# Yan-Xia/Text2Loc

Hardware: AMD Instinct MI355X
Metric: coarse-retrieval queries/sec over 11k-cell DB, embed_dim=256; top-1/3/5 recall parity (higher is better)
Workload: dtype f16; 1 GPU; KITTI360Pose-sized val DB: N=11259 cells x D=256 resident in HBM, Q=4096 precomputed text embeddings per step, top-10 (float64-exact ids); n_cells=11259, embed_dim=256, top_k=10, parallelism=single-gpu, layout=one resident DB, two launches per step (scan, re-rank)

## Files before the change

### text2loc_amd/csrc/capi.hip

```cpp
#include <limits.h>
#include <string.h>

#include "t2l_internal.h"

namespace t2l {

int fail(t2l_ctx* ctx, int code, const std::string& msg) {
  if (ctx) ctx->err = msg;
  return code;
}

void event_begin(t2l_ctx* ctx, const char* name, hipStream_t s) {
  if (!ctx->profile_events) return;
  EventRing& e = ctx->events[name];
  if (e.a.empty()) {
    e.a.resize(kEventRing);
    e.b.resize(kEventRing);
    for (int i = 0; i < kEventRing; ++i) {
      (void)hipEventCreate(&e.a[i]);
      (void)hipEventCreate(&e.b[i]);
    }
  }
  e.open = (e.calls++ % ctx->profile_events) == 0;
  if (e.open) (void)hipEventRecord(e.a[e.head], s);
// ... 315 lines not shown
  }
  return hipSuccess;
}

int t2l_search_fallbacks(t2l_ctx* ctx, int32_t* out_count) {
  if (!ctx || !out_count) return T2L_EINVAL;
  T2L_HIP(ctx, hipSetDevice(ctx->device));
  T2L_HIP(ctx, hipDeviceSynchronize());
  int32_t c[8];
  T2L_HIP(ctx, read_counters(ctx, c));
  *out_count = c[0] + (c[7] - c[6]);
  return T2L_OK;
}

#ifdef T2L_STAMPS
int t2l_debug_stamps(t2l_ctx* ctx, long long* out24) {
  T2L_HIP(ctx, hipDeviceSynchronize());
  T2L_HIP(ctx, hipMemcpy(out24, ctx->fb_count + 16, 24 * sizeof(long long), hipMemcpyDeviceToHost));
  const long long init[8] = {0, 0, 0, 0, LLONG_MAX, 0, LLONG_MAX, 0};
  T2L_HIP(ctx, hipMemcpy(ctx->fb_count + 16, init, sizeof(init), hipMemcpyHostToDevice));
  return T2L_OK;
}
#endif

int t2l_search_counters(t2l_ctx* ctx, int32_t* out8) {
  if (!ctx || !out8) return T2L_EINVAL;
  T2L_HIP(ctx, hipSetDevice(ctx->device));
  T2L_HIP(ctx, hipDeviceSynchronize());
  T2L_HIP(ctx, read_counters(ctx, out8));
  return T2L_OK;
}

int t2l_search_rescored(t2l_ctx* ctx, int32_t* out_count) {
// ... 342 lines not shown
```

### text2loc_amd/csrc/search.hip

```cpp
#include <float.h>
#include <limits.h>

#include <type_traits>

#include "t2l_internal.h"
#include "search_dev.h"

namespace t2l {

__device__ __forceinline__ void reset_counts(int32_t* fb_count, int32_t* fb_prev, int zero_counts, int tid) {
  if (zero_counts && tid < 16) {
    fb_count[64 + tid] = fb_prev[tid];
    fb_prev[tid] = 0;
  }
  if (!zero_counts && tid == 0) {
    fb_count[12] += fb_count[4];
    fb_count[4] = fb_count[6] = 0;
  }
}


__global__ __launch_bounds__(256) void split_db_kernel(const float* __restrict__ db, uint4* __restrict__ out, int rows) {
  const int gid = blockIdx.x * 256 + threadIdx.x;
  const int row = gid >> 5, c = gid & 31;
  if (row >= rows) return;
  const float4* src = reinterpret_cast<const float4*>(db + (size_t)row * kD + 8 * c);
  uint4 hi, lo;
  split8(src[0], src[1], hi, lo);
  out[(size_t)row * 64 + c] = hi;
  out[(size_t)row * 64 + 32 + c] = lo;
}

constexpr int kWideQPerWave = 64;
constexpr int kWideQPerBlock = 4 * kWideQPerWave;

template <int LL, int NBUF>
__global__ __launch_bounds__(256, 1) void scanw_kernel(const uint4* __restrict__ dbs, int n_rows, int n_tiles, int code_bits,
                                                       const float* __restrict__ q, int Q, int nsplit,
                                                       float* __restrict__ cand, int32_t* __restrict__ fb_count, int32_t* __restrict__ fb_prev,
                                                       int zero_counts, float pinf) {
  extern __shared__ __attribute__((aligned(16))) float smem[];
  const int tid = threadIdx.x, lane = tid & 63, wave = tid >> 6;
  const int half = lane >> 5, col = lane & 31;
  const int sp = blockIdx.x % nsplit, qb = blockIdx.x / nsplit;
  const int nt = sp < n_tiles ? (n_tiles - sp + nsplit - 1) / nsplit : 0;
  const int qrow0 = qb * kWideQPerBlock + wave * kWideQPerWave + col, qrow1 = qrow0 + 32;
  const int mask = ~((1 << code_bits) - 1);
  int vmask = mask;
  asm volatile("" : "+v"(vmask));
  if (blockIdx.x == 0) reset_counts(fb_count, fb_prev, zero_counts, tid);
  if (nt == 0) return;
  const int uwave = uniform_wave_id();

  auto dma_of = [&](int j, int buf) {
    const int tile = sp + min(j, nt - 1) * nsplit;
    WideDma d;
    d.src = reinterpret_cast<const char*>(dbs) + ((size_t)tile * kTileRows + uwave * 8) * 1024;
    d.dst = lds_addr_of(smem + buf * kTileFloats + uwave * 8 * kRowStrideF);
    d.lane16 = lane * 16;
    return d;
  };
#pragma unroll
  for (int b = 0; b < NBUF - 1; ++b) {
    const WideDma d = dma_of(b, b);
#pragma unroll
// ... 84 lines not shown
  if (pos >= rows_pad) return;
  const int row = plane_row(pos, n_rows);
  if (row >= n_rows) {
    out[gid] = make_uint4(0u, 0u, 0u, 0u);
    return;
  }
  int shift;
  half_shift_of(norms[1], shift);
  const float4* src = reinterpret_cast<const float4*>(db + (size_t)row * kD + 8 * c);
  const float4 a = src[0], b = src[1];
  out[gid] = make_uint4(pack_f16x2(a.x, a.y, shift), pack_f16x2(a.z, a.w, shift), pack_f16x2(b.x, b.y, shift),
                        pack_f16x2(b.z, b.w, shift));
}

template <int LL>
__global__ __launch_bounds__(256, 1) void scanh_kernel(const uint4* __restrict__ dbh, int n_rows, int n_tiles, int code_bits,
                                                       const float* __restrict__ q, int Q, int nsplit,
                                                       float* __restrict__ cand, int32_t* __restrict__ fb_count, int32_t* __restrict__ fb_prev,
                                                       int zero_counts, float pinf) {
  constexpr int NBUF = 4;
  extern __shared__ __attribute__((aligned(16))) float smem[];
  const int tid = threadIdx.x, lane = tid & 63;
  const int half = lane >> 5, col = lane & 31;
  const int sp = blockIdx.x % nsplit, qb = blockIdx.x / nsplit;
  const int nt = sp < n_tiles ? (n_tiles - sp + nsplit - 1) / nsplit : 0;
  const int uwave = uniform_wave_id();
  const int qrow0 = qb * kWideQPerBlock + uwave * kWideQPerWave + col, qrow1 = qrow0 + 32;
  const int mask = ~((1 << code_bits) - 1);
  int vmask = mask;
  asm volatile("" : "+v"(vmask));
  if (blockIdx.x == 0) reset_counts(fb_count, fb_prev, zero_counts, tid);
  if (nt == 0) return;

  const unsigned lds_base = lds_addr_of(smem);
  auto dma_of = [&](int j, int buf) {
    const int tile = sp + min(j, nt - 1) * nsplit;
    HalfDma d;
    d.src = reinterpret_cast<const char*>(dbh) + (size_t)tile * kHalfTileBytes + uwave * 4096;
    d.dst = lds_base + buf * kHalfTileBytes + uwave * 4096;
    d.lane16 = lane * 16;
    return d;
  };
#pragma unroll
  for (int b = 0; b < NBUF - 1; ++b) {
    const HalfDma d = dma_of(b, b);
#pragma unroll
// ... 100 lines not shown
  double* out_score;
  int32_t* flags;
  int32_t* fb_count;
  float eps_rel_probe, pinf;
  int n_rows, defer, stat_mode;
  int32_t* host_stat;
  int seq, wide_cap;
  int rec6;
  int slot_bits = 0;
};

constexpr int kMergedLL = 8;
#ifndef T2L_SEL_RD
#define T2L_SEL_RD 2
#endif
template <int LL, int NS, bool MERGE = false, int SEL = 0>
__global__ __launch_bounds__(512, 1) void scanp_kernel(const uint4* __restrict__ dbt, int n_rows, int n_tiles, int code_bits,
                                                       const float* __restrict__ q, int Q, int nsplit,
                                                       float* __restrict__ cand, int32_t* __restrict__ fb_count, int32_t* __restrict__ fb_prev,
                                                       int zero_counts, float pinf, unsigned long long* __restrict__ span,
                                                       unsigned span_seq, int xcd_qgroups, int slot_bits) {
  static_assert(NS == 4, "the step loop below is unrolled for a ring of 4 slots");
  constexpr bool EPI = SEL == 1;
  static_assert(!MERGE || LL == 6, "the in-workgroup list merge is written for lists of 6");
  static_assert(!SEL || MERGE, "the tile-local selection's dropped-bound leaves through the merged record's bound");
  extern __shared__ __attribute__((aligned(16))) float smem[];
  constexpr int kSlotBytes = 2 * kHalfTileBytes;
  constexpr unsigned kExchange = 2 * kSlotBytes;
  const int tid = threadIdx.x, lane = tid & 63;
  const int half = lane >> 5, col = lane & 31;
  int sp = blockIdx.x % nsplit, qb = blockIdx.x / nsplit;
  if (xcd_qgroups > 1) {
    const int GQ = xcd_qgroups, GS = 8 / GQ, nqb = gridDim.x / nsplit;
    const int x = blockIdx.x & 7, j = blockIdx.x >> 3, per = nqb / GQ;
    qb = (j % per) * GQ + x % GQ;
    sp = (j / per) * GS + x / GQ;
  }
  const int uwave = uniform_wave_id();
  const int quad = uwave >> 2, wq = uwave & 3;
  const int vn = 2 * nsplit, vs = sp + quad * nsplit;
  const int nt = vs < n_tiles ? (n_tiles - vs + vn - 1) / vn : 0;
  const int steps = sp < n_tiles ? (n_tiles - sp + vn - 1) / vn : 0;
  constexpr int kCS = MERGE ? 2 : 0;
  const int mask = ~((1 << (code_bits + kCS)) - 1);
  const int code_q = MERGE ? (quad << 1) : 0;
  int vmask = mask;
  asm volatile("" : "+v"(vmask));
  if (blockIdx.x == 0) reset_counts(fb_count, fb_prev, zero_counts, tid);
  if (steps == 0) return;
  const unsigned long long wg_t0 = __builtin_amdgcn_s_memrealtime();
#ifdef T2L_STAMPS
#define T2L_STAMP(k)                                                                                                   \
  if (tid == 0) {                                                                                                      \
    const long long t_ = __builtin_amdgcn_s_memrealtime();                                                             \
    if (blockIdx.x == 37) reinterpret_cast<long long*>(fb_count + 16)[k] = t_;                                         \
    if (k == 0) atomicMin(reinterpret_cast<unsigned long long*>(fb_count + 16) + 4, (unsigned long long)t_);           \
    if (k == 0) atomicMax(reinterpret_cast<unsigned long long*>(fb_count + 16) + 5, (unsigned long long)t_);           \
    if (k == 3) atomicMin(reinterpret_cast<unsigned long long*>(fb_count + 16) + 6, (unsigned long long)t_);           \
    if (k == 3) atomicMax(reinterpret_cast<unsigned long long*>(fb_count + 16) + 7, (unsigned long long)t_);           \
  }
#define T2L_STAMP2(k) if (tid == 0 && blockIdx.x == 37) reinterpret_cast<long long*>(fb_count + 32)[k] = __builtin_amdgcn_s_memrealtime()
#define T2L_STAMP3(k)                                                                                                  \
  {                                                                                                                    \
    __builtin_amdgcn_sched_barrier(0);                                                                                 \
    if (tid == 0 && blockIdx.x == 37) reinterpret_cast<long long*>(fb_count + 48)[k] = __builtin_amdgcn_s_memrealtime(); \
    __builtin_amdgcn_sched_barrier(0);                                                                                 \
  }
#else
#define T2L_STAMP(k)
#define T2L_STAMP2(k)
#define T2L_STAMP3(k)
#endif
  T2L_STAMP(0);

  const unsigned lds_base = lds_addr_of(smem);
  const unsigned lane16 = lane * 16;
  auto dma_of = [&](int i, int slot) {
    PairDma d;
    const int t0 = min(sp + (2 * i) * nsplit, n_tiles - 1), t1 = min(sp + (2 * i + 1) * nsplit, n_tiles - 1);
    d.src0 = reinterpret_cast<const char*>(dbt) + (size_t)t0 * kHalfTileBytes + uwave * 2048;
    d.src1 = reinterpret_cast<const char*>(dbt) + (size_t)t1 * kHalfTileBytes + uwave * 2048;
    d.dst = lds_base + slot * kSlotBytes + uwave * 2048;
    d.lane16 = lane16;
    return d;
  };
#pragma unroll
  for (int b = 0; b < 2; ++b) {
    const PairDma d = dma_of(b, b);
#pragma unroll
    for (int e = 0; e < 4; ++e) d.piece(e);
  }

  u32x4 q0[16], q1[16];
  {
    const int ql = tid >> 2, qt = tid & 3;
    char* ex_w = reinterpret_cast<char*>(smem) + kExchange + ql * 512;
    const char* ex_r = reinterpret_cast<const char*>(smem) + kExchange + (wq * 32 + col) * 512;
    float4 v[2][16];
#pragma unroll
    for (int g = 0; g < 2; ++g) {
      const int qrow = min(qb * kWideQPerBlock + (ql >> 5) * kWideQPerWave + g * 32 + (ql & 31), Q - 1);
      const float4* qp = reinterpret_cast<const float4*>(q + (size_t)qrow * kD) + qt;
#pragma unroll
      for (int i = 0; i < 16; ++i) v[g][i] = qp[4 * i];
#ifdef T2L_EXP_HALFLOAD
      if (g == 1) {
#pragma unroll
        for (int i = 0; i < 16; ++i) v[1][i] = v[0][i];
      }
#endif
    }
#pragma unroll
    for (int g = 0; g < 2; ++g) {
      float m = 0.f;
#pragma unroll
      for (int i = 0; i < 16; ++i) {
        m = fmaxf(fmaxf(m, fabsf(v[g][i].x)), fabsf(v[g][i].y));
        m = fmaxf(fmaxf(m, fabsf(v[g][i].z)), fabsf(v[g][i].w));
      }
      if (g == 0) { T2L_STAMP2(0); } else { T2L_STAMP2(3); }
      m = fmaxf(m, dpp_f<kDppXor1>(m));
      m = fmaxf(m, dpp_f<kDppXor2>(m));
      int shift;
      half_shift_of(m, shift);
      if (g == 1) __syncthreads();
#pragma unroll
      for (int j = 0; j < 16; ++j) {
        const float4 a = v[g][j];
        typedef unsigned u32x2 __attribute__((ext_vector_type(2)));
        *reinterpret_cast<u32x2*>(ex_w + (((2 * j + (qt >> 1)) ^ (ql & 31)) << 4) + ((qt & 1) << 3)) =
            u32x2{pack_f16x2(a.x, a.y, shift), pack_f16x2(a.z, a.w, shift)};
      }
      __syncthreads();
      if (g == 0) { T2L_STAMP2(1); } else { T2L_STAMP2(4); }
#pragma unroll
      for (int s = 0; s < 16; ++s) {
        const u32x4 f = *reinterpret_cast<const u32x4*>(ex_r + ((((half << 4) + s) ^ col) << 4));
        if (g == 0) q0[s] = pin_agpr(f); else q1[s] = pin_agpr(f);
      }
      if (g == 0) { T2L_STAMP2(2); } else { T2L_STAMP2(5); }
    }
    __syncthreads();
  }
  T2L_STAMP(1);
  {
    const PairDma d = dma_of(2, 2);
#pragma unroll
    for (int e = 0; e < 4; ++e) d.piece(e);
  }

  std::conditional_t<SEL != 0, TileSelLists<LL>, WideLists<LL>> w;
#pragma unroll
  for (int i = 0; i < LL; ++i) w.ls0[i] = w.ls1[i] = T2L_NEG_INF;
  if constexpr (SEL) w.dA0 = w.dB0 = w.dA1 = w.dB1 = w.t0 = w.t1 = w.t2 = w.k = T2L_NEG_INF;
  else w.key0 = w.key1 = T2L_NEG_INF;
  f32x16 accA0, accA1, accB0, accB1;
#pragma unroll
  for (int r = 0; r < 16; ++r) accA0[r] = accA1[r] = accB0[r] = accB1[r] = T2L_NEG_INF;
// ... 192 lines not shown
      T2L_STAMP3(5);
      const int qrow = qb * kWideQPerBlock + wq * kWideQPerWave + lane;
      if (qrow < Q) {
        float4* out = reinterpret_cast<float4*>(cand + ((size_t)qrow * nsplit + record_slot(sp, nsplit, slot_bits)) * kMergedLL);
        out[0] = make_float4(M[0], M[1], M[2], M[3]);
        out[1] = make_float4(M[4], M[5], M[6], M[7]);
      }
      T2L_STAMP3(6);
    }
  } else {
    put_list(qrow0, w.ls0);
    put_list(qrow1, w.ls1);
  }
  if (span && threadIdx.x == 0) {
    const unsigned long long t1 = __builtin_amdgcn_s_memrealtime(), tag = (unsigned long long)span_seq << 40, tm = (1ull << 40) - 1;
    *reinterpret_cast<ulonglong2*>(span + 2 * blockIdx.x) = make_ulonglong2(tag | (wg_t0 & tm), tag | (t1 & tm));
  }
  T2L_STAMP(3);
}

template <int NW>
struct WgExactSharedN {
  double score[NW][32];
  int row[NW][32];
};
typedef WgExactSharedN<4> WgExactShared;

constexpr int kWideCap = 1024;

__device__ __forceinline__ void top32_insert(double& ts, int& tr, double cd, int cr, int lane) {
  {
// ... 109 lines not shown

__device__ __forceinline__ void publish_report(const RerankArgs& a) {
  int32_t* fb_count = a.fb_count;
  if (a.host_stat && a.seq > 0) {
    a.host_stat[1] = fb_count[64 + 10] == 2 ? fb_count[64 + 3] : fb_count[64 + 2];
    a.host_stat[2] = fb_count[64 + 9];
    a.host_stat[3] = fb_count[64 + 0] + fb_count[64 + 4] + fb_count[64 + 12];
    a.host_stat[4] = fb_count[64 + 10];
    a.host_stat[5] = fb_count[64 + 10] == 2 ? fb_count[64 + 3] : fb_count[64 + 1];
    __hip_atomic_store(&a.host_stat[0], a.seq, __ATOMIC_RELEASE, __HIP_MEMORY_SCOPE_SYSTEM);
  }
  fb_count[9] = a.Q;
  fb_count[10] = a.stat_mode;
}

template <int LL, int L, bool MG = false>
__device__ __forceinline__ void rerank_query(const RerankArgs& a, const int qid, const int lane, int* my_wg_flag, int* wr_buf) {
  static_assert(!MG || LL == kMergedLL, "merged records are 8 floats");
  const float* __restrict__ db = a.db;
  const float* __restrict__ q = a.q;
  const int Q = a.Q, K = a.K, parts = a.parts, code_bits = a.code_bits, row_offset = a.row_offset, half_mode = a.half_mode;
  const int slack_bits = MG ? code_bits + 2 : code_bits;
  const int strided_rows = half_mode ? a.n_rows : 0;
  auto krow = [&](float key, int part) {
    if constexpr (MG) {
      const int b = __float_as_int(key), src = b & 3;
      return key_row(__int_as_float(b >> 2), 2 * (part + (src >> 1) * parts) + (src & 1), 2 * parts, code_bits, strided_rows);
    } else {
      return key_row(key, part, parts >> 1, code_bits, strided_rows);
    }
  };
  const float* __restrict__ cand = a.cand;
  const float eps_rel = a.eps_rel, eps_rel_probe = a.eps_rel_probe, pinf = a.pinf;
  const float* __restrict__ db_norm_max = a.db_norm_max;
  int32_t* __restrict__ out_idx = a.out_idx;
  double* __restrict__ out_score = a.out_score;
  int32_t* __restrict__ flags = a.flags;
  int32_t* __restrict__ fb_count = a.fb_count;
  const int n_rows = a.n_rows, defer = a.defer, wide_cap = a.wide_cap;

  float lst[LL];
  {
    const int mslot = MG ? record_slot(min(lane, parts - 1), parts, a.slot_bits) : min(lane, parts - 1);
    const float* mine = cand + ((size_t)qid * parts + mslot) * LL;
    if constexpr (MG) {
      const float4 v0 = reinterpret_cast<const float4*>(mine)[0], v1 = reinterpret_cast<const float4*>(mine)[1];
      lst[0] = v0.x; lst[1] = v0.y; lst[2] = v0.z; lst[3] = v0.w;
      lst[4] = v1.x; lst[5] = v1.y; lst[6] = v1.z; lst[7] = v1.w;
    } else if constexpr (LL % 2 == 0) {
#pragma unroll
      for (int i = 0; i < LL / 2; ++i) {
        const float2 v = reinterpret_cast<const float2*>(mine)[i];
        lst[2 * i] = v.x;
        lst[2 * i + 1] = v.y;
      }
    } else {
#pragma unroll
      for (int i = 0; i < LL; ++i) lst[i] = mine[i];
    }
    if (lane >= parts) {
#pragma unroll
      for (int i = 0; i < LL; ++i) lst[i] = T2L_NEG_INF;
    }
  }
  const float lane_floor = lst[LL - 1];
  if constexpr (MG) lst[LL - 1] = T2L_NEG_INF;
  float b1 = T2L_NEG_INF;
  if constexpr (MG) {
    if (a.rec6) {
      b1 = lst[LL - 2];
      lst[LL - 2] = T2L_NEG_INF;
    }
  }
  const float floor_max = wave_max_f32(fmaxf(lane_floor, b1), pinf);
  const int seg = lane & 15;
  double qd[16];
  float q_absmax = 0.f;
  {
    const float4* qp = reinterpret_cast<const float4*>(q + (size_t)qid * kD) + seg;
#pragma unroll
    for (int i = 0; i < 4; ++i) {
      const float4 v = qp[16 * i];
      qd[4 * i] = (double)v.x;
      qd[4 * i + 1] = (double)v.y;
      qd[4 * i + 2] = (double)v.z;
      qd[4 * i + 3] = (double)v.w;
      q_absmax = fmaxf(fmaxf(fmaxf(q_absmax, fabsf(v.x)), fabsf(v.y)), fmaxf(fabsf(v.z), fabsf(v.w)));
    }
  }

  float my_key = T2L_NEG_INF;
  int my_part = 0;
  auto merge_round = [&](int r) {
    const float bk = wave_max_f32(lst[0], pinf);
    const unsigned long long who = __ballot(lst[0] == bk);
    const int bl = __ffsll((long long)who) - 1;
    if (lane == r) {
      my_key = bk;
      my_part = bl;
    }
    const bool pop = lane == bl;
#pragma unroll
    for (int i = 0; i < LL - 1; ++i) lst[i] = pop ? lst[i + 1] : lst[i];
    lst[LL - 1] = pop ? T2L_NEG_INF : lst[LL - 1];
  };
#pragma unroll
  for (int r = 0; r < L - 4; ++r) merge_round(r);
  int my_row = (lane < L - 4 && my_key != T2L_NEG_INF) ? krow(my_key, my_part) : INT_MAX;

  double kscale = 1.0;
  bool representable = true;
  {
    const float m = row16_max_f32(q_absmax);
    int sq, sd;
    representable = half_shift_of(m, sq);
    representable = half_shift_of(db_norm_max[1], sd) && representable;
    if (half_mode) {
      kscale = ldexp(1.0, -(sq + sd));
    } else {
      representable = representable && abs(sq - 14) <= 40 && abs(sd - 14) <= 40;
    }
  }

  double qn = 0.0;
#pragma unroll
  for (int i = 0; i < 16; ++i) qn += qd[i] * qd[i];
  qn = row16_sum_f64(qn);
  const double eps32 = (double)eps_rel * sqrt(qn) * (double)(*db_norm_max);
  constexpr int LA = L - 4;
  float4 rows[L / 4][4];
  auto gather = [&](int p) {
    const int row = __shfl(my_row, 4 * p + (lane >> 4));
#ifdef T2L_EXP_RERANK_TWICE
    {
      const int other = row == INT_MAX ? 0 : (row * 7 + 13) % n_rows;
      const float4* op = reinterpret_cast<const float4*>(db + (size_t)other * kD) + seg;
#pragma unroll
      for (int i = 0; i < 4; ++i) {
        float4 v = op[16 * i];
        asm volatile("" ::"v"(v.x), "v"(v.y), "v"(v.z), "v"(v.w));
      }
    }
#endif
    const float4* rp = reinterpret_cast<const float4*>(db + (size_t)(row == INT_MAX ? 0 : row) * kD) + seg;
#pragma unroll
    for (int i = 0; i < 4; ++i) rows[p][i] = rp[16 * i];
  };
  double my_d = -__builtin_inf();
  auto score = [&](int p) {
    double d0 = 0.0, d1 = 0.0;
#pragma unroll
    for (int i = 0; i < 4; ++i) {
      d0 += (double)rows[p][i].x * qd[4 * i];
      d1 += (double)rows[p][i].y * qd[4 * i + 1];
      d0 += (double)rows[p][i].z * qd[4 * i + 2];
      d1 += (double)rows[p][i].w * qd[4 * i + 3];
    }
    const double d = row16_sum_f64(d0 + d1);
    const double mine = __shfl(d, 16 * (lane & 3));
    if ((lane >> 2) == p && lane < L && my_row != INT_MAX) my_d = mine;
  };
  auto rank_among = [&](auto n_tag) {
// ... 7 lines not shown
      const int ij = __builtin_amdgcn_readlane(my_row, j);
      r += (dj > my_d || (dj == my_d && ij < my_row)) ? 1 : 0;
    }
    return r;
  };
  auto emit = [&](bool ok, int r) {
    if (lane < K) {
      out_idx[(size_t)qid * K + lane] = -1;
      if (out_score) out_score[(size_t)qid * K + lane] = -__builtin_inf();
    }
    if (ok && r < K) {
      out_idx[(size_t)qid * K + r] = my_row + row_offset;
      if (out_score) out_score[(size_t)qid * K + r] = my_d;
    }
  };
#pragma unroll
  for (int p = 0; p < L / 4 - 1; ++p) gather(p);
#pragma unroll
  for (int p = 0; p < L / 4 - 1; ++p) score(p);
  bool early = false;
  if (K <= LA && representable && eps_rel_probe == 0.f) {
    const float gA = fmaxf(__uint_as_float(__builtin_amdgcn_readlane(__float_as_uint(my_key), LA - 1)), floor_max);
    if (gA != T2L_NEG_INF) {
      const int rA = rank_among(std::integral_constant<int, LA>{});
      const bool validA = lane < LA && my_row != INT_MAX;
      const unsigned long long kthA = __ballot(validA && rA == K - 1);
      if (kthA != 0ull) {
        const double dK = __shfl(my_d, __ffsll((long long)kthA) - 1);
        if (dK > (double)gA * kscale + key_slack(gA, slack_bits, eps32, kscale)) {
          emit(validA, rA);
          early = true;
        }
// ... 295 lines not shown
    }
  }
  }
  }
}

template <int LL, int L, bool MG = false>
__global__ __launch_bounds__(256, (MG ? 4 : 1)) void rerank_kernel(const float* __restrict__ db, const float* __restrict__ q, int Q,
                                                     int K, int parts, int code_bits,
                                                     const float* __restrict__ cand, int row_offset, float eps_rel,
                                                     const float* __restrict__ db_norm_max, int half_mode,
                                                     int32_t* __restrict__ out_idx, double* __restrict__ out_score,
                                                     int32_t* __restrict__ flags, int32_t* __restrict__ fb_count,
                                                     float eps_rel_probe, float pinf, int n_rows, int defer, int stat_mode,
                                                     int32_t* __restrict__ host_stat, int seq, int wide_cap, int rec6, int slot_bits) {
  __shared__ WgExactShared exact_sh;
  __shared__ int wg_flag[4];
  __shared__ int wide_rows[4][kWideCap];
  const RerankArgs a{db, q, Q, K, parts, code_bits, cand, row_offset, eps_rel, db_norm_max, half_mode, out_idx, out_score, flags, fb_count,
                     eps_rel_probe, pinf, n_rows, defer, stat_mode, host_stat, seq, wide_cap, rec6, slot_bits};
  const int lane = threadIdx.x & 63;
  const int qid = blockIdx.x * 4 + (threadIdx.x >> 6);
  if (threadIdx.x < 4) wg_flag[threadIdx.x] = 0;
  if (blockIdx.x == 0 && threadIdx.x == 0) publish_report(a);
  __syncthreads();
  if (qid < Q) rerank_query<LL, L, MG>(a, qid, lane, &wg_flag[threadIdx.x >> 6], wide_rows[threadIdx.x >> 6]);
  __syncthreads();
#pragma unroll 1
  for (int w = 0; w < 4; ++w) {
    if (!wg_flag[w]) continue;
    const int fq = blockIdx.x * 4 + w;
    if (threadIdx.x == 0) atomicAdd(&fb_count[0], 1);
    wg_exact_scan(db, n_rows, q + (size_t)fq * kD, K, row_offset, out_idx + (size_t)fq * K,
                  out_score ? out_score + (size_t)fq * K : nullptr, exact_sh);
  }
}

__global__ __launch_bounds__(256) void db_norm_kernel(const float* __restrict__ db, int n_rows, float* out) {
  __shared__ float red[4];
  __shared__ int red_a[4];
  const int lane = threadIdx.x & 63, wave = threadIdx.x >> 6;
// ... 93 lines not shown
                         bool first, bool pair, hipStream_t s) {
  const int n_tiles = (n_rows + kTileRows - 1) / kTileRows;
  const int parts = 2 * nsplit;
  const int zero = first;
  const int half_mode = ctx->eff_mode == 0;
  const bool probing = ctx->search_mode == 0 && ctx->eff_mode == 2;
  const double operand_eps = ctx->eff_mode == 0 ? 9.85e-4 : (ctx->eff_mode == 2 ? 2.0e-5 : 0.0);
  const float eps_rel = (float)(ctx->eps_scale * ((kD + 8) * 5.9604644775390625e-08 + operand_eps));
  const float eps_probe = probing ? (float)(ctx->eps_scale * ((kD + 8) * 5.9604644775390625e-08 + 9.85e-4)) : 0.f;
  const int stat_mode = probing ? 2 : (half_mode ? 1 : 0);
  const int seq = first ? ++ctx->stat_seq : 0;
  const int defer = ctx->heavy ? 1 : 0;
  bool merged = false;
  int rec_slot_bits = 0;
  if constexpr (LL <= 6) {
    const dim3 grid((Q + kWideQPerBlock - 1) / kWideQPerBlock * (nsplit / 2));
    const size_t lds = (size_t)4 * 2 * kHalfTileBytes + (size_t)256 * (kMergedLL + 3) * sizeof(float);
    static PerDeviceOnce once;
    if (once.need(ctx->device)) {
      allow_lds(&scanp_kernel<LL, 4>, lds);
      if constexpr (LL == 6) allow_lds(&scanp_kernel<LL, 4, true>, lds);
      if constexpr (LL == 6) allow_lds(&scanp_kernel<LL, 4, true, 1>, lds);
      if constexpr (LL == 6) allow_lds(&scanp_kernel<LL, 4, true, 2>, lds);
      once.mark(ctx->device);
    }
    const unsigned span_seq = ++ctx->span_seq;
    unsigned long long* span = ctx->scan_span && grid.x <= (unsigned)kSpanWgs ? ctx->scan_span + (size_t)2 * kSpanWgs * (span_seq % kSpanRing) : nullptr;
    if (ctx->span_grid) ctx->span_grid[span_seq % kSpanRing] = span ? grid.x : 0;
    int xq = ctx->xcd_qgroups;
    {
      const int nqb = (Q + kWideQPerBlock - 1) / kWideQPerBlock, ns = nsplit / 2;
      if (xq < 2 || 8 % xq || nqb % xq || ns % (8 / xq) || (nqb * ns) % 8) xq = 1;
    }
    int slot_bits = 0;
    if (ctx->search_epilogue && xq > 1)
      for (int gs = 8 / xq; gs > 1; gs >>= 1) ++slot_bits;
    rec_slot_bits = slot_bits;
    hipEvent_t ea, eb;
    const bool ev = event_pair(ctx, "search_scan", &ea, &eb);
    auto launch = [&](auto kern) {
      if (ev)
        hipExtLaunchKernelGGL(kern, grid, dim3(512), (uint32_t)lds, s, ea, eb, 0u, dbh, n_rows, n_tiles, code_bits, q, Q, nsplit / 2, ctx->cand_score,
                              ctx->fb_count, ctx->fb_prev, zero, __builtin_inff(), span, span_seq, xq, slot_bits);
      else
        hipLaunchKernelGGL(kern, grid, dim3(512), lds, s, dbh, n_rows, n_tiles, code_bits, q, Q, nsplit / 2, ctx->cand_score, ctx->fb_count,
                           ctx->fb_prev, zero, __builtin_inff(), span, span_seq, xq, slot_bits);
    };
    if constexpr (LL == 6 && L == 16) {
      merged = (ctx->search_merge == 1 || (ctx->search_merge == 2 && ctx->merge_live && !ctx->heavy)) && code_bits <= 9;
    }
    if constexpr (LL == 6) {
      if (merged && ctx->search_tile_sel && ctx->search_epilogue) launch(scanp_kernel<LL, 4, true, 1>);
      else if (merged && ctx->search_tile_sel) launch(scanp_kernel<LL, 4, true, 2>);
      else if (merged) launch(scanp_kernel<LL, 4, true>);
    }
    if (!merged) launch(scanp_kernel<LL, 4>);
  } else {
  event_begin(ctx, "search_scan", s);
  if (ctx->eff_mode == 0) {
    const dim3 grid((Q + kWideQPerBlock - 1) / kWideQPerBlock * nsplit);
    const size_t lds = (size_t)4 * kHalfTileBytes;
    static PerDeviceOnce once;
    if (once.need(ctx->device)) {
      allow_lds(&scanh_kernel<LL>, (size_t)4 * kHalfTileBytes);
      once.mark(ctx->device);
    }
    hipLaunchKernelGGL((scanh_kernel<LL>), grid, dim3(256), lds, s, dbh, n_rows, n_tiles, code_bits, q, Q, nsplit,
                       ctx->cand_score, ctx->fb_count, ctx->fb_prev, zero, __builtin_inff());
  } else if (ctx->eff_mode == 2) {
    const dim3 grid((Q + kWideQPerBlock - 1) / kWideQPerBlock * nsplit);
    const size_t lds = (size_t)4 * kTileFloats * sizeof(float);
    static PerDeviceOnce once;
    if (once.need(ctx->device)) {
      allow_lds(&scanw_kernel<LL, 4>, (size_t)4 * kTileFloats * sizeof(float));
      once.mark(ctx->device);
    }
    hipLaunchKernelGGL((scanw_kernel<LL, 4>), grid, dim3(256), lds, s, dbs, n_rows, n_tiles, code_bits, q, Q, nsplit,
                       ctx->cand_score, ctx->fb_count, ctx->fb_prev, zero, __builtin_inff());
  }
  event_end(ctx, "search_scan", s);
  }
  T2L_HIP(ctx, hipGetLastError());
  hipEvent_t ea, eb;
  if constexpr (LL == 6 && L == 16) {
    if (merged) {
      const bool evr = ctx->profile_rerank && event_pair(ctx, "search_rerank", &ea, &eb);
      if (evr)
        hipExtLaunchKernelGGL((rerank_kernel<kMergedLL, L, true>), dim3((Q + 3) / 4), dim3(256), 0u, s, ea, eb, 0u, db, q, Q, K, nsplit / 2,
                              code_bits, (const float*)ctx->cand_score, row_offset, eps_rel, (const float*)ctx->db_norm_max, half_mode, out_idx,
                              out_score, ctx->flags, ctx->fb_count, eps_probe, __builtin_inff(), n_rows, defer, stat_mode,
                              ctx->host_stat_dev, seq, min(ctx->wide_repair, kWideCap), ctx->search_tile_sel ? 1 : 0, rec_slot_bits);
      else
// ... 226 lines not shown
```

### text2loc_amd/csrc/search_dev.h

```cpp
#pragma once
#include <float.h>
#include <limits.h>

#include "t2l_internal.h"

namespace t2l {

typedef float f32x16 __attribute__((ext_vector_type(16)));

#define T2L_NEG_INF (-__builtin_inff())

template <int L, int I = L - 1>
__device__ __forceinline__ void ins_key(float (&s)[L], float x) {
  if constexpr (I == 0) {
    s[0] = __builtin_amdgcn_fmed3f(s[0], x, __builtin_inff());
  } else {
    s[I] = __builtin_amdgcn_fmed3f(s[I - 1], s[I], x);
    ins_key<L, I - 1>(s, x);
  }
}

__device__ __forceinline__ float make_key(float v, int mask, int code) {
  return __int_as_float((__float_as_int(v) & mask) | code);
}
// ... 489 lines not shown
```

Baseline: 101.1 million queries/s.

## Overlap scan prologue loads, use 2D/3D grids, and prefetch rerank inputs early

The scan kernels now take a 2D or 3D grid with precomputed tiles-per-split quotient and remainder, which removes the per-block integer division and modulo and the XCD remapping arithmetic. The merged scan kernel issues query loads with explicit vmcnt waits, half of them into AGPRs, interleaved with the first DB tile DMAs, and it defers the counter reset until after that prologue. The rerank kernel prefetches the query row and norm values alongside the candidate lists, drops the leading __syncthreads, and moves publish_report after the per-query work. Optional timestamp instrumentation is also added. The hand-written waitcnt values and AGPR placement are fragile if the instruction mix changes.

```diff
diff --git a/text2loc_amd/csrc/capi.hip b/text2loc_amd/csrc/capi.hip
--- a/text2loc_amd/csrc/capi.hip
+++ b/text2loc_amd/csrc/capi.hip
@@ -353,9 +353,9 @@
 }
 
 #ifdef T2L_STAMPS
-int t2l_debug_stamps(t2l_ctx* ctx, long long* out24) {
+int t2l_debug_stamps(t2l_ctx* ctx, long long* out48) {
   T2L_HIP(ctx, hipDeviceSynchronize());
-  T2L_HIP(ctx, hipMemcpy(out24, ctx->fb_count + 16, 24 * sizeof(long long), hipMemcpyDeviceToHost));
+  T2L_HIP(ctx, hipMemcpy(out48, ctx->fb_count + 16, 48 * sizeof(long long), hipMemcpyDeviceToHost));
   const long long init[8] = {0, 0, 0, 0, LLONG_MAX, 0, LLONG_MAX, 0};
   T2L_HIP(ctx, hipMemcpy(ctx->fb_count + 16, init, sizeof(init), hipMemcpyHostToDevice));
   return T2L_OK;
diff --git a/text2loc_amd/csrc/search.hip b/text2loc_amd/csrc/search.hip
--- a/text2loc_amd/csrc/search.hip
+++ b/text2loc_amd/csrc/search.hip
@@ -35,20 +35,20 @@
 constexpr int kWideQPerBlock = 4 * kWideQPerWave;
 
 template <int LL, int NBUF>
-__global__ __launch_bounds__(256, 1) void scanw_kernel(const uint4* __restrict__ dbs, int n_rows, int n_tiles, int code_bits,
+__global__ __launch_bounds__(256, 1) void scanw_kernel(const uint4* __restrict__ dbs, int n_rows, int tiles_q, int tiles_r, int code_bits,
                                                        const float* __restrict__ q, int Q, int nsplit,
                                                        float* __restrict__ cand, int32_t* __restrict__ fb_count, int32_t* __restrict__ fb_prev,
                                                        int zero_counts, float pinf) {
   extern __shared__ __attribute__((aligned(16))) float smem[];
   const int tid = threadIdx.x, lane = tid & 63, wave = tid >> 6;
   const int half = lane >> 5, col = lane & 31;
-  const int sp = blockIdx.x % nsplit, qb = blockIdx.x / nsplit;
-  const int nt = sp < n_tiles ? (n_tiles - sp + nsplit - 1) / nsplit : 0;
+  const int sp = blockIdx.x, qb = blockIdx.y;
+  const int nt = tiles_q + (sp < tiles_r ? 1 : 0);
   const int qrow0 = qb * kWideQPerBlock + wave * kWideQPerWave + col, qrow1 = qrow0 + 32;
   const int mask = ~((1 << code_bits) - 1);
   int vmask = mask;
   asm volatile("" : "+v"(vmask));
-  if (blockIdx.x == 0) reset_counts(fb_count, fb_prev, zero_counts, tid);
+  if ((blockIdx.x | blockIdx.y) == 0) reset_counts(fb_count, fb_prev, zero_counts, tid);
   if (nt == 0) return;
   const int uwave = uniform_wave_id();
 
@@ -163,7 +163,7 @@
 }
 
 template <int LL>
-__global__ __launch_bounds__(256, 1) void scanh_kernel(const uint4* __restrict__ dbh, int n_rows, int n_tiles, int code_bits,
+__global__ __launch_bounds__(256, 1) void scanh_kernel(const uint4* __restrict__ dbh, int n_rows, int tiles_q, int tiles_r, int code_bits,
                                                        const float* __restrict__ q, int Q, int nsplit,
                                                        float* __restrict__ cand, int32_t* __restrict__ fb_count, int32_t* __restrict__ fb_prev,
                                                        int zero_counts, float pinf) {
@@ -171,14 +171,14 @@
   extern __shared__ __attribute__((aligned(16))) float smem[];
   const int tid = threadIdx.x, lane = tid & 63;
   const int half = lane >> 5, col = lane & 31;
-  const int sp = blockIdx.x % nsplit, qb = blockIdx.x / nsplit;
-  const int nt = sp < n_tiles ? (n_tiles - sp + nsplit - 1) / nsplit : 0;
+  const int sp = blockIdx.x, qb = blockIdx.y;
+  const int nt = tiles_q + (sp < tiles_r ? 1 : 0);
   const int uwave = uniform_wave_id();
   const int qrow0 = qb * kWideQPerBlock + uwave * kWideQPerWave + col, qrow1 = qrow0 + 32;
   const int mask = ~((1 << code_bits) - 1);
   int vmask = mask;
   asm volatile("" : "+v"(vmask));
-  if (blockIdx.x == 0) reset_counts(fb_count, fb_prev, zero_counts, tid);
+  if ((blockIdx.x | blockIdx.y) == 0) reset_counts(fb_count, fb_prev, zero_counts, tid);
   if (nt == 0) return;
 
   const unsigned lds_base = lds_addr_of(smem);
@@ -309,12 +309,39 @@
 #ifndef T2L_SEL_RD
 #define T2L_SEL_RD 2
 #endif
+#ifdef T2L_STAMPS
+#define T2L_STAMP(k)                                                                                                   \
+  if (tid == 0) {                                                                                                      \
+    const long long t_ = __builtin_amdgcn_s_memrealtime();                                                             \
+    if (wg == 37) reinterpret_cast<long long*>(fb_count + 16)[k] = t_;                                                 \
+    if (k == 0) atomicMin(reinterpret_cast<unsigned long long*>(fb_count + 16) + 4, (unsigned long long)t_);           \
+    if (k == 0) atomicMax(reinterpret_cast<unsigned long long*>(fb_count + 16) + 5, (unsigned long long)t_);           \
+    if (k == 3) atomicMin(reinterpret_cast<unsigned long long*>(fb_count + 16) + 6, (unsigned long long)t_);           \
+    if (k == 3) atomicMax(reinterpret_cast<unsigned long long*>(fb_count + 16) + 7, (unsigned long long)t_);           \
+  }
+#define T2L_STAMP2(k) if (tid == 0 && wg == 37) reinterpret_cast<long long*>(fb_count + 32)[k] = __builtin_amdgcn_s_memrealtime()
+#define T2L_STAMP2_AT(k, t) if (tid == 0 && wg == 37) reinterpret_cast<long long*>(fb_count + 32)[k] = (long long)(t)
+#define T2L_STAMP3(k)                                                                                                  \
+  {                                                                                                                    \
+    __builtin_amdgcn_sched_barrier(0);                                                                                 \
+    if (tid == 0 && wg == 37) reinterpret_cast<long long*>(fb_count + 48)[k] = __builtin_amdgcn_s_memrealtime();       \
+    __builtin_amdgcn_sched_barrier(0);                                                                                 \
+  }
+#else
+#define T2L_STAMP(k)
+#define T2L_STAMP2(k)
+#define T2L_STAMP2_AT(k, t)
+#define T2L_STAMP3(k)
+#endif
+
 template <int LL, int NS, bool MERGE = false, int SEL = 0>
-__global__ __launch_bounds__(512, 1) void scanp_kernel(const uint4* __restrict__ dbt, int n_rows, int n_tiles, int code_bits,
-                                                       const float* __restrict__ q, int Q, int nsplit,
-                                                       float* __restrict__ cand, int32_t* __restrict__ fb_count, int32_t* __restrict__ fb_prev,
-                                                       int zero_counts, float pinf, unsigned long long* __restrict__ span,
-                                                       unsigned span_seq, int xcd_qgroups, int slot_bits) {
+__global__ __launch_bounds__(512, 1) void scanp_kernel(const float* __restrict__ q, const uint4* __restrict__ dbt, int Q, int nsplit,
+                                                       int tiles_q, int tiles_r, int n_tiles, int lgq, int grid_y, int code_bits,
+                                                       int zero_counts, float pinf, int n_rows, unsigned span_seq, int slot_bits,
+                                                       float* __restrict__ cand, int32_t* __restrict__ fb_count,
+                                                       int32_t* __restrict__ fb_prev, unsigned long long* __restrict__ span) {
+  const unsigned long long wg_t0 = __builtin_amdgcn_s_memrealtime();
+  asm volatile("" ::"s"(dbt), "s"(q), "s"(grid_y));
   static_assert(NS == 4, "the step loop below is unrolled for a ring of 4 slots");
   constexpr bool EPI = SEL == 1;
   static_assert(!MERGE || LL == 6, "the in-workgroup list merge is written for lists of 6");
@@ -324,49 +351,20 @@
   constexpr unsigned kExchange = 2 * kSlotBytes;
   const int tid = threadIdx.x, lane = tid & 63;
   const int half = lane >> 5, col = lane & 31;
-  int sp = blockIdx.x % nsplit, qb = blockIdx.x / nsplit;
-  if (xcd_qgroups > 1) {
-    const int GQ = xcd_qgroups, GS = 8 / GQ, nqb = gridDim.x / nsplit;
-    const int x = blockIdx.x & 7, j = blockIdx.x >> 3, per = nqb / GQ;
-    qb = (j % per) * GQ + x % GQ;
-    sp = (j / per) * GS + x / GQ;
-  }
+  const int qb = (blockIdx.y << lgq) + (blockIdx.x & ((1 << lgq) - 1));
+  const int sp = blockIdx.z * (8 >> lgq) + (blockIdx.x >> lgq);
+  const int wg = blockIdx.x + (lgq ? 8 : nsplit) * (blockIdx.y + grid_y * blockIdx.z);
   const int uwave = uniform_wave_id();
   const int quad = uwave >> 2, wq = uwave & 3;
   const int vn = 2 * nsplit, vs = sp + quad * nsplit;
-  const int nt = vs < n_tiles ? (n_tiles - vs + vn - 1) / vn : 0;
-  const int steps = sp < n_tiles ? (n_tiles - sp + vn - 1) / vn : 0;
+  const int nt = tiles_q + (vs < tiles_r ? 1 : 0);
+  const int steps = tiles_q + (sp < tiles_r ? 1 : 0);
   constexpr int kCS = MERGE ? 2 : 0;
   const int mask = ~((1 << (code_bits + kCS)) - 1);
   const int code_q = MERGE ? (quad << 1) : 0;
   int vmask = mask;
   asm volatile("" : "+v"(vmask));
-  if (blockIdx.x == 0) reset_counts(fb_count, fb_prev, zero_counts, tid);
   if (steps == 0) return;
-  const unsigned long long wg_t0 = __builtin_amdgcn_s_memrealtime();
-#ifdef T2L_STAMPS
-#define T2L_STAMP(k)                                                                                                   \
-  if (tid == 0) {                                                                                                      \
-    const long long t_ = __builtin_amdgcn_s_memrealtime();                                                             \
-    if (blockIdx.x == 37) reinterpret_cast<long long*>(fb_count + 16)[k] = t_;                                         \
-    if (k == 0) atomicMin(reinterpret_cast<unsigned long long*>(fb_count + 16) + 4, (unsigned long long)t_);           \
-    if (k == 0) atomicMax(reinterpret_cast<unsigned long long*>(fb_count + 16) + 5, (unsigned long long)t_);           \
-    if (k == 3) atomicMin(reinterpret_cast<unsigned long long*>(fb_count + 16) + 6, (unsigned long long)t_);           \
-    if (k == 3) atomicMax(reinterpret_cast<unsigned long long*>(fb_count + 16) + 7, (unsigned long long)t_);           \
-  }
-#define T2L_STAMP2(k) if (tid == 0 && blockIdx.x == 37) reinterpret_cast<long long*>(fb_count + 32)[k] = __builtin_amdgcn_s_memrealtime()
-#define T2L_STAMP3(k)                                                                                                  \
-  {                                                                                                                    \
-    __builtin_amdgcn_sched_barrier(0);                                                                                 \
-    if (tid == 0 && blockIdx.x == 37) reinterpret_cast<long long*>(fb_count + 48)[k] = __builtin_amdgcn_s_memrealtime(); \
-    __builtin_amdgcn_sched_barrier(0);                                                                                 \
-  }
-#else
-#define T2L_STAMP(k)
-#define T2L_STAMP2(k)
-#define T2L_STAMP3(k)
-#endif
-  T2L_STAMP(0);
 
   const unsigned lds_base = lds_addr_of(smem);
   const unsigned lane16 = lane * 16;
@@ -379,34 +377,48 @@
     d.lane16 = lane16;
     return d;
   };
-#pragma unroll
-  for (int b = 0; b < 2; ++b) {
-    const PairDma d = dma_of(b, b);
-#pragma unroll
-    for (int e = 0; e < 4; ++e) d.piece(e);
-  }
-
   u32x4 q0[16], q1[16];
+  int parked;
   {
     const int ql = tid >> 2, qt = tid & 3;
     char* ex_w = reinterpret_cast<char*>(smem) + kExchange + ql * 512;
     const char* ex_r = reinterpret_cast<const char*>(smem) + kExchange + (wq * 32 + col) * 512;
-    float4 v[2][16];
+    f32x4 v[2][16];
+    auto load_q = [&](auto agpr_tag, f32x4& dst, const float4* p, auto off_tag) {
+      constexpr int OFF = decltype(off_tag)::value;
+      if constexpr (decltype(agpr_tag)::value) asm volatile("global_load_dwordx4 %0, %1, off offset:%2" : "=a"(dst) : "v"(p), "n"(OFF) : "memory");
+      else asm volatile("global_load_dwordx4 %0, %1, off offset:%2" : "=&v"(dst) : "v"(p), "n"(OFF) : "memory");
+    };
+    auto row_ptr = [&](int g) {
+      const int qrow = min(qb * kWideQPerBlock + (ql >> 5) * kWideQPerWave + g * 32 + (ql & 31), Q - 1);
+      return reinterpret_cast<const float4*>(q + (size_t)qrow * kD) + qt;
+    };
+    const float4 *qp0 = row_ptr(0), *qp1 = row_ptr(1);
+    T2L_STAMP(0);
+    static_for<0, 16>([&](auto i) { load_q(std::false_type{}, v[0][i], qp0, std::integral_constant<int, 64 * decltype(i)::value>{}); });
+#pragma unroll
+    for (int b = 0; b < 2; ++b) {
+      const PairDma d = dma_of(b, b);
+#pragma unroll
+      for (int e = 0; e < 4; ++e) d.piece(e);
+    }
+    static_for<0, 16>([&](auto i) { load_q(std::true_type{}, v[1][i], qp1, std::integral_constant<int, 64 * decltype(i)::value>{}); });
+    parked = fb_prev[tid & 15];
+    auto landed = [&](int g) {
+      if (g == 0) {
+        asm volatile("s_waitcnt vmcnt(25)" ::: "memory");
+#pragma unroll
+        for (int i = 0; i < 16; ++i) asm volatile("" : "+v"(v[0][i]));
+      } else {
+        asm volatile("s_waitcnt vmcnt(0)" ::: "memory");
+#pragma unroll
+        for (int i = 0; i < 16; ++i) asm volatile("" : "+a"(v[1][i]));
+        asm volatile("" : "+v"(parked));
+      }
+    };
 #pragma unroll
     for (int g = 0; g < 2; ++g) {
-      const int qrow = min(qb * kWideQPerBlock + (ql >> 5) * kWideQPerWave + g * 32 + (ql & 31), Q - 1);
-      const float4* qp = reinterpret_cast<const float4*>(q + (size_t)qrow * kD) + qt;
-#pragma unroll
-      for (int i = 0; i < 16; ++i) v[g][i] = qp[4 * i];
-#ifdef T2L_EXP_HALFLOAD
-      if (g == 1) {
-#pragma unroll
-        for (int i = 0; i < 16; ++i) v[1][i] = v[0][i];
-      }
-#endif
-    }
-#pragma unroll
-    for (int g = 0; g < 2; ++g) {
+      landed(g);
       float m = 0.f;
 #pragma unroll
       for (int i = 0; i < 16; ++i) {
@@ -421,7 +433,7 @@
       if (g == 1) __syncthreads();
 #pragma unroll
       for (int j = 0; j < 16; ++j) {
-        const float4 a = v[g][j];
+        const f32x4 a = v[g][j];
         typedef unsigned u32x2 __attribute__((ext_vector_type(2)));
         *reinterpret_cast<u32x2*>(ex_w + (((2 * j + (qt >> 1)) ^ (ql & 31)) << 4) + ((qt & 1) << 3)) =
             u32x2{pack_f16x2(a.x, a.y, shift), pack_f16x2(a.z, a.w, shift)};
@@ -437,6 +449,14 @@
     }
     __syncthreads();
   }
+  if (wg == 0) {
+    if (zero_counts && tid < 16) {
+      fb_count[64 + tid] = parked;
+      fb_prev[tid] = 0;
+    }
+    if (!zero_counts) reset_counts(fb_count, fb_prev, 0, tid);
+  }
+  T2L_STAMP2_AT(6, wg_t0);
   T2L_STAMP(1);
   {
     const PairDma d = dma_of(2, 2);
@@ -659,7 +679,7 @@
   }
   if (span && threadIdx.x == 0) {
     const unsigned long long t1 = __builtin_amdgcn_s_memrealtime(), tag = (unsigned long long)span_seq << 40, tm = (1ull << 40) - 1;
-    *reinterpret_cast<ulonglong2*>(span + 2 * blockIdx.x) = make_ulonglong2(tag | (wg_t0 & tm), tag | (t1 & tm));
+    *reinterpret_cast<ulonglong2*>(span + 2 * wg) = make_ulonglong2(tag | (wg_t0 & tm), tag | (t1 & tm));
   }
   T2L_STAMP(3);
 }
@@ -799,6 +819,21 @@
   fb_count[10] = a.stat_mode;
 }
 
+#ifdef T2L_STAMPS
+constexpr int kRerankStampWg = 513;
+#define T2L_RSTAMP_AT(k, t) if (qid == 4 * kRerankStampWg && lane == 0) reinterpret_cast<long long*>(a.fb_count + 96)[k] = (long long)(t)
+#define T2L_RSTAMP(k, ...)                                                                                              \
+  {                                                                                                                    \
+    __builtin_amdgcn_sched_barrier(0);                                                                                 \
+    asm volatile(__VA_ARGS__);                                                                                         \
+    T2L_RSTAMP_AT(k, __builtin_amdgcn_s_memrealtime());                                                                \
+    __builtin_amdgcn_sched_barrier(0);                                                                                 \
+  }
+#else
+#define T2L_RSTAMP_AT(k, t)
+#define T2L_RSTAMP(k, ...)
+#endif
+
 template <int LL, int L, bool MG = false>
 __device__ __forceinline__ void rerank_query(const RerankArgs& a, const int qid, const int lane, int* my_wg_flag, int* wr_buf) {
   static_assert(!MG || LL == kMergedLL, "merged records are 8 floats");
@@ -825,9 +860,13 @@
   const int n_rows = a.n_rows, defer = a.defer, wide_cap = a.wide_cap;
 
   float lst[LL];
+  const int seg = lane & 15;
+  float4 qraw[4];
+  float db_norm, db_absmax;
   {
     const int mslot = MG ? record_slot(min(lane, parts - 1), parts, a.slot_bits) : min(lane, parts - 1);
     const float* mine = cand + ((size_t)qid * parts + mslot) * LL;
+    const float4* qp = reinterpret_cast<const float4*>(q + (size_t)qid * kD) + seg;
     if constexpr (MG) {
       const float4 v0 = reinterpret_cast<const float4*>(mine)[0], v1 = reinterpret_cast<const float4*>(mine)[1];
       lst[0] = v0.x; lst[1] = v0.y; lst[2] = v0.z; lst[3] = v0.w;
@@ -843,6 +882,13 @@
 #pragma unroll
       for (int i = 0; i < LL; ++i) lst[i] = mine[i];
     }
+#pragma unroll
+    for (int i = 0; i < 4; ++i) qraw[i] = qp[16 * i];
+    db_norm = db_norm_max[0];
+    db_absmax = db_norm_max[1];
+    __builtin_amdgcn_sched_barrier(0);
+    T2L_RSTAMP(1, "");
+    T2L_RSTAMP(2, "s_waitcnt vmcnt(%0)" ::"n"(4));
     if (lane >= parts) {
 #pragma unroll
       for (int i = 0; i < LL; ++i) lst[i] = T2L_NEG_INF;
@@ -858,22 +904,6 @@
     }
   }
   const float floor_max = wave_max_f32(fmaxf(lane_floor, b1), pinf);
-  const int seg = lane & 15;
-  double qd[16];
-  float q_absmax = 0.f;
-  {
-    const float4* qp = reinterpret_cast<const float4*>(q + (size_t)qid * kD) + seg;
-#pragma unroll
-    for (int i = 0; i < 4; ++i) {
-      const float4 v = qp[16 * i];
-      qd[4 * i] = (double)v.x;
-      qd[4 * i + 1] = (double)v.y;
-      qd[4 * i + 2] = (double)v.z;
-      qd[4 * i + 3] = (double)v.w;
-      q_absmax = fmaxf(fmaxf(fmaxf(q_absmax, fabsf(v.x)), fabsf(v.y)), fmaxf(fabsf(v.z), fabsf(v.w)));
-    }
-  }
-
   float my_key = T2L_NEG_INF;
   int my_part = 0;
   auto merge_round = [&](int r) {
@@ -893,44 +923,65 @@
   for (int r = 0; r < L - 4; ++r) merge_round(r);
   int my_row = (lane < L - 4 && my_key != T2L_NEG_INF) ? krow(my_key, my_part) : INT_MAX;
 
+  T2L_RSTAMP(3, "");
+  constexpr int LA = L - 4;
+  float4 rows[L / 4][4];
+  auto gather = [&](int p) {
+    const int r0 = __builtin_amdgcn_readlane(my_row, 4 * p), r1 = __builtin_amdgcn_readlane(my_row, 4 * p + 1);
+    const int r2 = __builtin_amdgcn_readlane(my_row, 4 * p + 2), r3 = __builtin_amdgcn_readlane(my_row, 4 * p + 3);
+    const int grp = lane >> 4;
+    const int row = grp == 0 ? r0 : (grp == 1 ? r1 : (grp == 2 ? r2 : r3));
+#ifdef T2L_EXP_RERANK_TWICE
+    {
+      const int other = row == INT_MAX ? 0 : (row * 7 + 13) % n_rows;
+      const float4* op = reinterpret_cast<const float4*>(db + (size_t)other * kD) + seg;
+#pragma unroll
+      for (int i = 0; i < 4; ++i) {
+        float4 v = op[16 * i];
+        asm volatile("" ::"v"(v.x), "v"(v.y), "v"(v.z), "v"(v.w));
+      }
+    }
+#endif
+    const float4* rp = reinterpret_cast<const float4*>(db + (size_t)(row == INT_MAX ? 0 : row) * kD) + seg;
+#pragma unroll
+    for (int i = 0; i < 4; ++i) rows[p][i] = rp[16 * i];
+  };
+#pragma unroll
+  for (int p = 0; p < L / 4 - 1; ++p) {
+    gather(p);
+    if (p == 0) { T2L_RSTAMP(4, ""); }
+  }
+  __builtin_amdgcn_sched_barrier(0);
+
+  double qd[16];
+  float q_absmax = 0.f;
+#pragma unroll
+  for (int i = 0; i < 4; ++i) {
+    const float4 v = qraw[i];
+    qd[4 * i] = (double)v.x;
+    qd[4 * i + 1] = (double)v.y;
+    qd[4 * i + 2] = (double)v.z;
+    qd[4 * i + 3] = (double)v.w;
+    q_absmax = fmaxf(fmaxf(fmaxf(q_absmax, fabsf(v.x)), fabsf(v.y)), fmaxf(fabsf(v.z), fabsf(v.w)));
+  }
   double kscale = 1.0;
   bool representable = true;
   {
     const float m = row16_max_f32(q_absmax);
     int sq, sd;
     representable = half_shift_of(m, sq);
-    representable = half_shift_of(db_norm_max[1], sd) && representable;
+    representable = half_shift_of(db_absmax, sd) && representable;
     if (half_mode) {
       kscale = ldexp(1.0, -(sq + sd));
     } else {
       representable = representable && abs(sq - 14) <= 40 && abs(sd - 14) <= 40;
     }
   }
-
   double qn = 0.0;
 #pragma unroll
   for (int i = 0; i < 16; ++i) qn += qd[i] * qd[i];
   qn = row16_sum_f64(qn);
-  const double eps32 = (double)eps_rel * sqrt(qn) * (double)(*db_norm_max);
-  constexpr int LA = L - 4;
-  float4 rows[L / 4][4];
-  auto gather = [&](int p) {
-    const int row = __shfl(my_row, 4 * p + (lane >> 4));
-#ifdef T2L_EXP_RERANK_TWICE
-    {
-      const int other = row == INT_MAX ? 0 : (row * 7 + 13) % n_rows;
-      const float4* op = reinterpret_cast<const float4*>(db + (size_t)other * kD) + seg;
-#pragma unroll
-      for (int i = 0; i < 4; ++i) {
-        float4 v = op[16 * i];
-        asm volatile("" ::"v"(v.x), "v"(v.y), "v"(v.z), "v"(v.w));
-      }
-    }
-#endif
-    const float4* rp = reinterpret_cast<const float4*>(db + (size_t)(row == INT_MAX ? 0 : row) * kD) + seg;
-#pragma unroll
-    for (int i = 0; i < 4; ++i) rows[p][i] = rp[16 * i];
-  };
+  const double eps32 = (double)eps_rel * sqrt(qn) * (double)db_norm;
   double my_d = -__builtin_inf();
   auto score = [&](int p) {
     double d0 = 0.0, d1 = 0.0;
@@ -968,8 +1019,7 @@
       if (out_score) out_score[(size_t)qid * K + r] = my_d;
     }
   };
-#pragma unroll
-  for (int p = 0; p < L / 4 - 1; ++p) gather(p);
+  T2L_RSTAMP(5, "s_waitcnt vmcnt(%0)" ::"n"(4 * (L / 4 - 2)));
 #pragma unroll
   for (int p = 0; p < L / 4 - 1; ++p) score(p);
   bool early = false;
@@ -1295,6 +1345,9 @@
                                                      int32_t* __restrict__ flags, int32_t* __restrict__ fb_count,
                                                      float eps_rel_probe, float pinf, int n_rows, int defer, int stat_mode,
                                                      int32_t* __restrict__ host_stat, int seq, int wide_cap, int rec6, int slot_bits) {
+#ifdef T2L_STAMPS
+  const long long t_entry = __builtin_amdgcn_s_memrealtime();
+#endif
   __shared__ WgExactShared exact_sh;
   __shared__ int wg_flag[4];
   __shared__ int wide_rows[4][kWideCap];
@@ -1302,10 +1355,12 @@
                      eps_rel_probe, pinf, n_rows, defer, stat_mode, host_stat, seq, wide_cap, rec6, slot_bits};
   const int lane = threadIdx.x & 63;
   const int qid = blockIdx.x * 4 + (threadIdx.x >> 6);
-  if (threadIdx.x < 4) wg_flag[threadIdx.x] = 0;
+  asm volatile("" ::"s"(q), "s"(cand), "s"(db_norm_max), "s"(half_mode));
+  if (lane == 0) wg_flag[threadIdx.x >> 6] = 0;
+  T2L_RSTAMP_AT(0, t_entry);
+  if (qid < Q) rerank_query<LL, L, MG>(a, qid, lane, &wg_flag[threadIdx.x >> 6], wide_rows[threadIdx.x >> 6]);
+  T2L_RSTAMP(6, "");
   if (blockIdx.x == 0 && threadIdx.x == 0) publish_report(a);
-  __syncthreads();
-  if (qid < Q) rerank_query<LL, L, MG>(a, qid, lane, &wg_flag[threadIdx.x >> 6], wide_rows[threadIdx.x >> 6]);
   __syncthreads();
 #pragma unroll 1
   for (int w = 0; w < 4; ++w) {
@@ -1429,7 +1484,8 @@
   bool merged = false;
   int rec_slot_bits = 0;
   if constexpr (LL <= 6) {
-    const dim3 grid((Q + kWideQPerBlock - 1) / kWideQPerBlock * (nsplit / 2));
+    const int nqb = (Q + kWideQPerBlock - 1) / kWideQPerBlock, ns = nsplit / 2;
+    const unsigned n_wgs = (unsigned)(nqb * ns);
     const size_t lds = (size_t)4 * 2 * kHalfTileBytes + (size_t)256 * (kMergedLL + 3) * sizeof(float);
     static PerDeviceOnce once;
     if (once.need(ctx->device)) {
@@ -1440,13 +1496,15 @@
       once.mark(ctx->device);
     }
     const unsigned span_seq = ++ctx->span_seq;
-    unsigned long long* span = ctx->scan_span && grid.x <= (unsigned)kSpanWgs ? ctx->scan_span + (size_t)2 * kSpanWgs * (span_seq % kSpanRing) : nullptr;
-    if (ctx->span_grid) ctx->span_grid[span_seq % kSpanRing] = span ? grid.x : 0;
+    unsigned long long* span = ctx->scan_span && n_wgs <= (unsigned)kSpanWgs ? ctx->scan_span + (size_t)2 * kSpanWgs * (span_seq % kSpanRing) : nullptr;
+    if (ctx->span_grid) ctx->span_grid[span_seq % kSpanRing] = span ? n_wgs : 0;
     int xq = ctx->xcd_qgroups;
-    {
-      const int nqb = (Q + kWideQPerBlock - 1) / kWideQPerBlock, ns = nsplit / 2;
-      if (xq < 2 || 8 % xq || nqb % xq || ns % (8 / xq) || (nqb * ns) % 8) xq = 1;
-    }
+    if (xq < 2 || 8 % xq || nqb % xq || ns % (8 / xq) || (nqb * ns) % 8) xq = 1;
+    int lgq = 0;
+    while ((1 << lgq) < xq) ++lgq;
+    const dim3 grid = xq > 1 ? dim3(8, nqb / xq, ns / (8 / xq)) : dim3(ns, nqb, 1);
+    if (grid.y > 65535u || grid.z > 65535u) return fail(ctx, T2L_EINVAL, "t2l_search: more than 65,535 query blocks in one call");
+    const int vn = 2 * ns, tiles_q = n_tiles / vn, tiles_r = n_tiles % vn;
     int slot_bits = 0;
     if (ctx->search_epilogue && xq > 1)
       for (int gs = 8 / xq; gs > 1; gs >>= 1) ++slot_bits;
@@ -1455,11 +1513,11 @@
     const bool ev = event_pair(ctx, "search_scan", &ea, &eb);
     auto launch = [&](auto kern) {
       if (ev)
-        hipExtLaunchKernelGGL(kern, grid, dim3(512), (uint32_t)lds, s, ea, eb, 0u, dbh, n_rows, n_tiles, code_bits, q, Q, nsplit / 2, ctx->cand_score,
-                              ctx->fb_count, ctx->fb_prev, zero, __builtin_inff(), span, span_seq, xq, slot_bits);
+        hipExtLaunchKernelGGL(kern, grid, dim3(512), (uint32_t)lds, s, ea, eb, 0u, q, dbh, Q, ns, tiles_q, tiles_r, n_tiles, lgq, (int)grid.y,
+                              code_bits, zero, __builtin_inff(), n_rows, span_seq, slot_bits, ctx->cand_score, ctx->fb_count, ctx->fb_prev, span);
       else
-        hipLaunchKernelGGL(kern, grid, dim3(512), lds, s, dbh, n_rows, n_tiles, code_bits, q, Q, nsplit / 2, ctx->cand_score, ctx->fb_count,
-                           ctx->fb_prev, zero, __builtin_inff(), span, span_seq, xq, slot_bits);
+        hipLaunchKernelGGL(kern, grid, dim3(512), lds, s, q, dbh, Q, ns, tiles_q, tiles_r, n_tiles, lgq, (int)grid.y, code_bits, zero,
+                           __builtin_inff(), n_rows, span_seq, slot_bits, ctx->cand_score, ctx->fb_count, ctx->fb_prev, span);
     };
     if constexpr (LL == 6 && L == 16) {
       merged = (ctx->search_merge == 1 || (ctx->search_merge == 2 && ctx->merge_live && !ctx->heavy)) && code_bits <= 9;
@@ -1473,24 +1531,24 @@
   } else {
   event_begin(ctx, "search_scan", s);
   if (ctx->eff_mode == 0) {
-    const dim3 grid((Q + kWideQPerBlock - 1) / kWideQPerBlock * nsplit);
+    const dim3 grid(nsplit, (Q + kWideQPerBlock - 1) / kWideQPerBlock);
     const size_t lds = (size_t)4 * kHalfTileBytes;
     static PerDeviceOnce once;
     if (once.need(ctx->device)) {
       allow_lds(&scanh_kernel<LL>, (size_t)4 * kHalfTileBytes);
       once.mark(ctx->device);
     }
-    hipLaunchKernelGGL((scanh_kernel<LL>), grid, dim3(256), lds, s, dbh, n_rows, n_tiles, code_bits, q, Q, nsplit,
+    hipLaunchKernelGGL((scanh_kernel<LL>), grid, dim3(256), lds, s, dbh, n_rows, n_tiles / nsplit, n_tiles % nsplit, code_bits, q, Q, nsplit,
                        ctx->cand_score, ctx->fb_count, ctx->fb_prev, zero, __builtin_inff());
   } else if (ctx->eff_mode == 2) {
-    const dim3 grid((Q + kWideQPerBlock - 1) / kWideQPerBlock * nsplit);
+    const dim3 grid(nsplit, (Q + kWideQPerBlock - 1) / kWideQPerBlock);
     const size_t lds = (size_t)4 * kTileFloats * sizeof(float);
     static PerDeviceOnce once;
     if (once.need(ctx->device)) {
       allow_lds(&scanw_kernel<LL, 4>, (size_t)4 * kTileFloats * sizeof(float));
       once.mark(ctx->device);
     }
-    hipLaunchKernelGGL((scanw_kernel<LL, 4>), grid, dim3(256), lds, s, dbs, n_rows, n_tiles, code_bits, q, Q, nsplit,
+    hipLaunchKernelGGL((scanw_kernel<LL, 4>), grid, dim3(256), lds, s, dbs, n_rows, n_tiles / nsplit, n_tiles % nsplit, code_bits, q, Q, nsplit,
                        ctx->cand_score, ctx->fb_count, ctx->fb_prev, zero, __builtin_inff());
   }
   event_end(ctx, "search_scan", s);
diff --git a/text2loc_amd/csrc/search_dev.h b/text2loc_amd/csrc/search_dev.h
--- a/text2loc_amd/csrc/search_dev.h
+++ b/text2loc_amd/csrc/search_dev.h
@@ -2,11 +2,22 @@
 #include <float.h>
 #include <limits.h>
 
+#include <type_traits>
+
 #include "t2l_internal.h"
 
 namespace t2l {
 
 typedef float f32x16 __attribute__((ext_vector_type(16)));
+typedef float f32x4 __attribute__((ext_vector_type(4)));
+
+template <int FROM, int TO, class F>
+__device__ __forceinline__ void static_for(F&& f) {
+  if constexpr (FROM < TO) {
+    f(std::integral_constant<int, FROM>{});
+    static_for<FROM + 1, TO>(f);
+  }
+}
 
 #define T2L_NEG_INF (-__builtin_inff())
 
```

Measured after the change: 101.5 million queries/s (median of 4 runs). About the same (+0.5%).
